# nmoehrle/mvs-texturing

Hardware: AMD Instinct MI355X
Metric: faces/sec through view-selection (data-cost + MRF) (higher is better)
Workload: dtype f32

## Files before the change

### mvs-texturing_amd/csrc/api.hip

```cpp
#include "ctx.h"

#include <atomic>
#include <cmath>
#include <cstdio>
#include <cstdlib>
#include <cstring>
#include <chrono>
#include <mutex>
#include <string>
#include <thread>
#include <vector>

namespace mvs {
void dc_phase1(mvs_ctx* ctx, const mvs_settings* st);
void dc_phase2(mvs_ctx* ctx);
void dc_phase3(mvs_ctx* ctx, mvs_dc_stats* stats);
void undistort_image(mvs_ctx* ctx, const uint8_t* d_src, uint8_t* d_dst, int w, int h, double flen, double d0, double d1);
void dc_prune_labels(mvs_ctx* ctx, uint32_t kmax);
void dc_postprocess(mvs_ctx* ctx, uint32_t nf, uint32_t n_views, const uint32_t* h_ptr, const uint16_t* h_view_rev, const float* h_q_rev, const float* h_col_rev, const mvs_settings* st);
void mrf_setup(mvs_ctx* ctx, const mvs_mrf_params* params);
void mrf_sweep(mvs_ctx* ctx, uint32_t nb0, uint32_t ne0);
void mrf_energy(mvs_ctx* ctx, bool best, uint32_t nb0, uint32_t ne0, bool reduce = true);
void mrf_keep_best(mvs_ctx* ctx);
void mrf_exact_costs(mvs_ctx* ctx, uint32_t nb0, uint32_t ne0);
// ... 311 lines not shown
    if (!ctx) return fail(MVS_ERR_INVALID, "ctx is null");
    MVS_API_BEGIN
    MVS_HIP(hipStreamSynchronize(ctx->stream));
    if (ctx->own_stream && ctx->stream) MVS_HIP(hipStreamDestroy(ctx->stream));
    ctx->stream = (hipStream_t)hip_stream; ctx->own_stream = false;
    MVS_API_END
}

mvs_status mvs_ctx_synchronize(mvs_ctx* ctx) {
    if (!ctx) return fail(MVS_ERR_INVALID, "ctx is null");
    MVS_API_BEGIN
    MVS_HIP(hipStreamSynchronize(ctx->stream));
    MVS_API_END
}

mvs_status mvs_set_option(mvs_ctx* ctx, const char* name, int64_t value) {
    if (!ctx || !name) return fail(MVS_ERR_INVALID, "null argument");
    const std::string n(name);
    if (n == "count_rays") ctx->count_rays = value != 0;
    else if (n == "stats") ctx->stats = value != 0;
    else if (n == "verbose") ctx->verbose = value != 0;
    else if (n == "info_wave_area") ctx->info_wave_area = (int)std::max<int64_t>(0, std::min<int64_t>(value, 1 << 30));
    else if (n == "info_wave_area_words") ctx->info_wave_area_words = (int)std::max<int64_t>(1, std::min<int64_t>(value, 1 << 30));
    else if (n == "info_words") ctx->info_words = value != 0;
    else if (n == "info_cert_shift") ctx->info_cert_shift = (int)std::max<int64_t>(0, std::min<int64_t>(value, 40));
    else if (n == "max_labels") { if (value < 0 || value > 65535) return fail(MVS_ERR_INVALID, "max_labels: 0 (off) .. 65535"); ctx->max_labels = (int)value; }
    else if (n == "profile") ctx->profile = value != 0;
    else if (n == "prep_fused") ctx->prep_fused = value != 0;
    else if (n == "ray_xcd") ctx->ray_xcd = (int)value;
    else if (n == "mrf_xcd") ctx->mrf_xcd = (int)value;
    else if (n == "mrf_lag") ctx->mrf_lag = (int)value;
    else if (n == "shard_peer_push") ctx->shard_peer_push = value != 0;
    else if (n == "mrf_force_generic") ctx->mrf_force_generic = value != 0;
    else if (n == "mrf_wide") ctx->mrf_wide = value != 0;
    else if (n == "mrf_graph") ctx->mrf_graph = value != 0;
    else if (n == "mrf_late_old") ctx->mrf_late_old = (int)value;
    else if (n == "mrf_damp_period") ctx->mrf_damp_period = (int)std::max<int64_t>(0, std::min<int64_t>(value, 64));
    else if (n == "mrf_run_pad") ctx->mrf_run_pad = (value == 16) ? 16 : 4;
    else if (n == "mrf_blocks_per_cu") ctx->mrf_blocks_per_cu = std::max(0, (int)value);
    else if (n == "bvh_caller_order") ctx->bvh_caller_order = value != 0;
    else if (n == "dc_overlap_prep") ctx->dc_overlap_prep = value != 0;
    else if (n == "bvh_upper_min_faces") { ctx->kd_disabled = false; ctx->bvh_upper_min_faces = (uint32_t)std::max<int64_t>(0, std::min<int64_t>(value, 0xFFFFFFFFll)); ctx->order_pinned = false; }
    else if (n == "bvh_window") { ctx->kd_disabled = false; ctx->bvh_window = (uint32_t)std::max<int64_t>(0, std::min<int64_t>(value, 0x40000000)); ctx->order_pinned = false; }
    else if (n == "face_order") { ctx->face_order = value != 0 ? 1 : 0; ctx->order_pinned = false; }
    else return fail(MVS_ERR_INVALID, "unknown option " + n);
    return MVS_OK;
}

mvs_status mvs_ctx_get_profile(mvs_ctx* ctx, char* buf, size_t buf_size) {
    if (!ctx || !buf || buf_size < 3) return fail(MVS_ERR_INVALID, "null argument");
    MVS_API_BEGIN
    MVS_HIP(hipStreamSynchronize(ctx->stream));
    std::vector<std::string> names; std::vector<double> ms; std::vector<int> cnt;
    for (auto& sp : ctx->prof_spans) {
        float t = 0.0f;
        MVS_HIP(hipEventElapsedTime(&t, sp.a, sp.b));
        size_t k = 0;
        for (; k < names.size(); ++k) if (names[k] == sp.name) break;
        if (k == names.size()) { names.push_back(sp.name); ms.push_back(0.0); cnt.push_back(0); }
        ms[k] += t; cnt[k] += 1;
        if (sp.owns_a) ctx->prof_pool.push_back(sp.a);
        ctx->prof_pool.push_back(sp.b);
    }
    ctx->prof_spans.clear();
    std::string out = "{";
    for (size_t k = 0; k < names.size(); ++k) {
// ... 636 lines not shown
```

### mvs-texturing_amd/csrc/ctx.h

```cpp
#pragma once
#include <hip/hip_runtime.h>
#include <stdint.h>
#include <string.h>
#include <algorithm>
#include <stdexcept>
#include <string>
#include <vector>

#include "../../include/mvs_viewsel.h"
#include "dmath.h"

namespace mvs {

struct HipError : std::runtime_error {
    explicit HipError(const std::string& m) : std::runtime_error(m) {}
};
struct StatusError : std::runtime_error {
    mvs_status st;
    StatusError(mvs_status s, const std::string& m) : std::runtime_error(m), st(s) {}
};

#define MVS_HIP(expr)                                                                          \
    do {                                                                                       \
        hipError_t _e = (expr);                                                                \
// ... 157 lines not shown
    const uint32_t* r_ptr = nullptr; const uint16_t* r_view = nullptr; const float* r_cost = nullptr;
    bool csr_q_valid = false;
    bool have_costs = false;
    mvs_settings dc_settings{}; mvs_dc_stats dc_stats{}; int dc_phase = 0;

    mvs::DBuf<unsigned long long> g_keys, g_keys2; mvs::DBuf<uint32_t> g_vals, g_vals2, g_pos, g_cnt, g_adj_ptr, g_adj, g_faces; mvs::DBuf<float> g_normals;
    uint64_t g_adj_entries = 0; bool have_adj = false;

    mvs::DBuf<uint32_t> p_label_ptr, p_comp_ptr, p_comp_faces, p_parent, p_root, p_state, p_flag, p_pos, p_roots, p_roots2, p_rlab, p_rlab2, p_adj_ptr, p_adj, p_labels;

    mvs::DBuf<uint32_t> rg_parent, rg_root, rg_size, rg_bestl, rg_lose, rg_flag, rg_pos, rg_cstart, rg_have, rg_cfirst, rg_name;
    mvs::DBuf<unsigned long long> rg_gain, rg_cur, rg_key, rg_key2, rg_ck, rg_sum; mvs::DBuf<long long> rg_cgain; mvs::DBuf<uint2> rg_cut;

    mvs::DBuf<uint32_t> m_adj_ptr, m_adj, a_stage_ptr, a_stage; const uint32_t* r_adj_ptr = nullptr; const uint32_t* r_adj = nullptr;
    uint32_t r_adj_edges = 0; bool r_adj_edges_known = false;
    mvs::DBuf<mvs::NodeDesc> m_desc; mvs::DBuf<uint8_t> m_ident; mvs::DBuf<uint32_t> m_rec; uint64_t m_rec_words = 0; bool m_fast = false; int mrf_blocks_per_cu = 0 , mrf_xcd = 1, mrf_late_old = 1, mrf_run_pad = 4;
    mvs::DBuf<mvs::MrfEdge> m_edge; mvs::DBuf<uint32_t> m_size, m_rev ; mvs::DBuf<uint16_t> m_map;
    mvs::DBuf<uint8_t> m_msg_a;
    mvs::DBuf<uint32_t> m_sel, m_sel2, m_cand; mvs::DBuf<float> m_gain;
    mvs::DBuf<uint32_t> m_lab; mvs::DBuf<float> m_cost;
    uint32_t m_stride = 0;
    bool exact_valid = false; uint32_t exact_nb = 0, exact_ne = 0;
    uint32_t* b_sel = nullptr; uint32_t* b_lab = nullptr; float* b_cost = nullptr; bool best_resolved = false;
    mvs::DBuf<unsigned long long> m_energy; mvs::DBuf<uint32_t> m_moved; mvs::DBuf<uint32_t> m_alist; bool icm_dirty_valid = false;
    uint32_t m_n_adj = 0;
    uint32_t m_energy_blocks = 0;
    bool m_energy_from_sweep = false;
    uint64_t m_total = 0; uint32_t m_kmax = 0, m_degmax = 0;
    mvs::DBuf<uint32_t> m_colour, m_perm, m_tmp_a, m_tmp_b, m_tmp_c, m_sub; mvs::DBuf<uint8_t> m_cls; uint32_t m_colours = 0, m_n_fast = 0; std::vector<uint32_t> m_sub_begin;
    const uint32_t* m_colour_in = nullptr;
    const uint8_t* m_bnd = nullptr;
    int mrf_damp_period = 4;
    int mrf_force_generic = 0;
    int mrf_wide = 1;
    bool m_wide_layout = false;
    uint32_t m_range_nb = 0, m_range_ne = 0; std::vector<uint32_t> m_range_q;
    uint32_t m_sweep_no = 0;
    mvs_mrf_params m_params{};
    static constexpr uint32_t RING = 16;
    static constexpr uint32_t ICM_RING = 8;
    uint32_t* h_icm = nullptr; uint32_t* d_icm = nullptr; uint32_t icm_seq = 0;
    mvs::DBuf<mvs_mrf_progress> m_state; mvs::DBuf<unsigned long long> m_hist; mvs::DBuf<uint32_t> m_ctl;
    int mrf_graph = 1; hipStream_t cap_stream = nullptr; hipGraphExec_t sweep_exec = nullptr; uint32_t graph_launches = 0, graph_updates = 0, graph_instantiations = 0;
    mvs_mrf_progress* h_ring = nullptr; mvs_mrf_progress* d_ring = nullptr ; uint32_t steps_issued = 0; int mrf_lag = 1;
    int shard_peer_push = 1;
    uint32_t* h_seq = nullptr; uint32_t* d_seq = nullptr; uint32_t seq_base = 0;
};

namespace mvs {
struct Prof {
    mvs_ctx* c; size_t idx; bool on;
    Prof(mvs_ctx* ctx, const char* name) : c(ctx), idx(0), on(ctx->profile) {
        if (!on) return;
        auto get = [&]() { hipEvent_t e; if (!c->prof_pool.empty()) { e = c->prof_pool.back(); c->prof_pool.pop_back(); } else { MVS_HIP(hipEventCreate(&e)); } return e; };
        ProfSpan sp{name, get(), get(), true};
        MVS_HIP(hipEventRecord(sp.a, c->stream));
        idx = c->prof_spans.size(); c->prof_spans.push_back(sp);
    }
    void end() { if (on) { MVS_HIP(hipEventRecord(c->prof_spans[idx].b, c->stream)); on = false; } }
    ~Prof() { if (on) (void)hipEventRecord(c->prof_spans[idx].b, c->stream); }
};
struct ProfChain {
    mvs_ctx* c; hipEvent_t prev; bool on;
    static hipEvent_t get(mvs_ctx* c) { hipEvent_t e; if (!c->prof_pool.empty()) { e = c->prof_pool.back(); c->prof_pool.pop_back(); } else { MVS_HIP(hipEventCreate(&e)); } return e; }
    explicit ProfChain(mvs_ctx* ctx) : c(ctx), prev(nullptr), on(ctx->profile) {}
    void begin() { if (on && !prev) { prev = get(c); MVS_HIP(hipEventRecord(prev, c->stream)); first = true; } }
// ... 22 lines not shown
```

### mvs-texturing_amd/csrc/k_mrf.hip

```cpp
#include "ctx.h"
#include <rocprim/rocprim.hpp>
#include <atomic>

namespace mvs {

namespace {

constexpr uint16_t MAP_NONE = 0xFFFF;
constexpr uint32_t MSG_BASE = MVS_MRF_MSG_BASE;

typedef uint8_t msg_t;
struct MsgQ { float scale, step; };
__device__ __forceinline__ MsgQ msg_q(float lam) { return MsgQ{255.0f / lam, lam / 255.0f}; }
template <class T> __device__ __forceinline__ T ld_off(const void* base, uint32_t byte_off) { return *reinterpret_cast<const T*>(reinterpret_cast<const char*>(base) + byte_off); }
template <class T> __device__ __forceinline__ void st_off(void* base, uint32_t byte_off, T v) { *reinterpret_cast<T*>(reinterpret_cast<char*>(base) + byte_off) = v; }
__device__ __forceinline__ float min_raw(float a, float b) { float r; asm("v_min_f32 %0, %1, %2" : "=v"(r) : "v"(a), "v"(b)); return r; }
template <bool DAMP>
__device__ __forceinline__ uint32_t msg_pack_s(float raw_s, float alpha, float old_code, uint32_t byte, uint32_t word) {
    return __builtin_amdgcn_cvt_pk_u8_f32(DAMP ? __builtin_fmaf(old_code, alpha, raw_s) : raw_s, byte, word);
}
template <bool DAMP>
__device__ __forceinline__ uint32_t msg_pack(float raw, float oms, float alpha, float old_code, uint32_t byte, uint32_t word) {
    const float v = DAMP ? __builtin_fmaf(old_code, alpha, raw * oms) : raw * oms;
    return __builtin_amdgcn_cvt_pk_u8_f32(v, byte, word);
// ... 318 lines not shown
}

__global__ void __launch_bounds__(256) mrf_ident_kernel(const uint32_t* __restrict__ col_ptr, const uint16_t* __restrict__ view_id, const uint32_t* __restrict__ adj_ptr,
                                                        const uint32_t* __restrict__ adj, uint32_t F, const MrfEdge* __restrict__ edge, const uint8_t* __restrict__ cls,
                                                        uint8_t* __restrict__ ident) {
    const uint32_t i = (blockIdx.x * blockDim.x + threadIdx.x) >> 4;
    const uint32_t gl = threadIdx.x & 15;
    if (i >= F || cls[i] == CLS_GENERIC) return;
    const uint32_t p0 = col_ptr[i], K = col_ptr[i + 1] - p0;
    const uint32_t e0 = adj_ptr[i], e1 = adj_ptr[i + 1];
    for (uint32_t e = e0; e < e1; e += 3) {
        uint32_t kj[3], q0[3];
#pragma unroll
        for (int k = 0; k < 3; ++k) {
            const bool on = e + k < e1;
            kj[k] = on ? edge[e + k].kj : 0u;
            q0[k] = col_ptr[on ? adj[e + k] : i];
        }
        uint32_t same = 0;
#pragma unroll
        for (int k = 0; k < 3; ++k) same |= (kj[k] != 0u && kj[k] == K) ? (1u << k) : 0u;
        if (same) {
            for (uint32_t t = gl; t < K; t += 16) {
                const uint32_t v = view_id[p0 + t];
#pragma unroll
                for (int k = 0; k < 3; ++k)
                    if ((same >> k) & 1u) { if (view_id[q0[k] + t] != v) same &= ~(1u << k); }
            }
            for (int o = 8; o > 0; o >>= 1) same &= __shfl_xor(same, o, 16);
        }
        if (gl < 3 && e + gl < e1 && kj[gl] != 0u) ident[e + gl] = (uint8_t)((same >> gl) & 1u);
    }
}
__global__ void mrf_recsize_kernel(const uint32_t* __restrict__ col_ptr, const uint32_t* __restrict__ adj_ptr, const MrfEdge* __restrict__ edge,
                                   const uint8_t* __restrict__ ident, const uint8_t* __restrict__ cls, const uint32_t* __restrict__ perm, uint32_t F, uint32_t wide,
                                   uint32_t* __restrict__ rsz, uint32_t* __restrict__ qpos) {
    const uint32_t q = blockIdx.x * blockDim.x + threadIdx.x;
    if (q > F) return;
    uint32_t w = 0;
    if (q < F) {
        const uint32_t i = perm[q], K = col_ptr[i + 1] - col_ptr[i];
        qpos[i] = q;
        if (K && cls[i] != CLS_GENERIC) {
            w = (K + 3u) & ~3u;
            const bool w8 = wide != 0u && cls[i] == 1u;
            const uint32_t e0 = adj_ptr[i], e1 = adj_ptr[i + 1];
            for (uint32_t eb = e0; eb < e1; eb += 4) {
                uint32_t kj[4], id[4];
#pragma unroll
                for (int t = 0; t < 4; ++t) { const bool on = eb + t < e1; kj[t] = on ? edge[eb + t].kj : 0u; id[t] = on ? ident[eb + t] : 1u; }
#pragma unroll
                for (int t = 0; t < 4; ++t) if (kj[t] && !id[t]) w += w8 ? 2u * ((kj[t] + 7u) >> 3) : (kj[t] + 3u) >> 2;
            }
            w = (w + 3u) & ~3u;
        }
    }
    rsz[q] = w;
}
__global__ void __launch_bounds__(256) mrf_record_kernel(const uint32_t* __restrict__ col_ptr, const uint16_t* __restrict__ view_id, const float* __restrict__ cost,
                                                         const uint32_t* __restrict__ adj_ptr, const uint32_t* __restrict__ adj, const MrfEdge* __restrict__ edge,
                                                         const uint8_t* __restrict__ ident, const uint8_t* __restrict__ cls, const uint32_t* __restrict__ qpos, const uint32_t* __restrict__ roff,
                                                         uint32_t F, uint32_t wide, uint32_t* __restrict__ rec) {
    __shared__ uint16_t s_l[16][256];
    const uint32_t i = (blockIdx.x * blockDim.x + threadIdx.x) >> 4;
    const uint32_t gl = threadIdx.x & 15;
    if (i >= F) return;
    const uint32_t p0 = col_ptr[i], K = col_ptr[i + 1] - p0;
    const uint32_t ci = cls[i];
    if (K == 0 || ci == CLS_GENERIC) return;
    const bool w8 = wide != 0u && ci == 1u;
    const uint32_t rs = w8 ? 8u : 8u << ci, none_byte = w8 ? 64u : (ci < 3u ? 4u * rs : 0xFFu);
    const uint32_t lmask = w8 ? 7u : 3u, lshift = w8 ? 3u : 2u;
    const uint32_t q = qpos[i];
    uint16_t* tile = s_l[threadIdx.x >> 4];
    uint32_t* out = rec + REC_BASE + roff[q];
    const uint32_t K4 = (K + 3u) & ~3u;
    const uint32_t e0 = adj_ptr[i], deg = adj_ptr[i + 1] - e0;
    uint32_t kj3[3], q03[3];
    {
        uint32_t kj[3], idn[3], nb[3];
#pragma unroll
        for (uint32_t d = 0; d < 3; ++d) { const bool on = d < deg; kj[d] = on ? edge[e0 + d].kj : 0u; idn[d] = on ? (uint32_t)ident[e0 + d] : 1u; nb[d] = on ? adj[e0 + d] : i; }
#pragma unroll
// ... 595 lines not shown
        bool stop = false;
        if ((int)sw >= min_sweeps && (int)sw > window) {
            const unsigned long long prev = hist[sw - (uint32_t)window];
            stop = (double)(prev - p.best) < (double)min_improvement * (double)prev;
        }
        if ((int)sw >= max_sweeps) stop = true;
        if (stop) { p.stopped = 1u; p.stop_sweep = sw; }
    }
    *st = p;
    const uint32_t n = ctl[0] + 1u; ctl[0] = n;
    if (ring) {
        const uint32_t slot = n % ring_slots;
        ring[slot] = p;
        __threadfence_system();
        __hip_atomic_store(ring_seq + slot, ctl[1] + n, __ATOMIC_RELEASE, __HIP_MEMORY_SCOPE_SYSTEM);
    }
}
__global__ void report_u32_kernel(const uint32_t* __restrict__ src, uint32_t* __restrict__ dst, uint32_t* __restrict__ dst_seq, uint32_t seq) {
    *dst = *src;
    __threadfence_system();
    __hip_atomic_store(dst_seq, seq, __ATOMIC_RELEASE, __HIP_MEMORY_SCOPE_SYSTEM);
}
__global__ void report_words_kernel(const uint32_t* __restrict__ src, uint32_t n, uint32_t* __restrict__ dst, uint32_t* __restrict__ dst_seq, uint32_t seq) {
    if (threadIdx.x < n) dst[threadIdx.x] = src[threadIdx.x];
    __threadfence_system();
    __syncthreads();
    if (threadIdx.x == 0) __hip_atomic_store(dst_seq, seq, __ATOMIC_RELEASE, __HIP_MEMORY_SCOPE_SYSTEM);
}
__global__ void mrf_flip_kernel(mvs_mrf_progress* __restrict__ st) { st->best_w = st->w; st->w ^= 1u; }

}

constexpr uint32_t EPART_BLOCKS = 2048;

void mrf_setup(mvs_ctx* ctx, const mvs_mrf_params* params) {
    hipStream_t s = ctx->stream;
    const uint32_t F = ctx->csr_faces;
    ctx->m_params = *params;
    if (!(params->rho > 0.0f && params->rho <= 1.0f) || !(params->damping >= 0.0f && params->damping < 1.0f))
        throw StatusError(MVS_ERR_INVALID, "mrf params: need 0 < rho <= 1, 0 <= damping < 1");
    if (params->window < 1 || params->min_sweeps < 0 || !(params->min_improvement >= 0.0f) || params->icm_iters < 0)
        throw StatusError(MVS_ERR_INVALID, "mrf params: need window >= 1, min_sweeps >= 0, min_improvement >= 0, icm_iters >= 0");
    uint32_t E = ctx->r_adj_edges;
    if (!ctx->r_adj_edges_known) {
        MVS_HIP(hipMemcpyAsync(&E, ctx->r_adj_ptr + F, sizeof(uint32_t), hipMemcpyDeviceToHost, s));
        MVS_HIP(hipStreamSynchronize(s));
    }
    ctx->m_size.ensure((size_t)E + 2); ctx->m_edge.ensure((size_t)E + 1); ctx->m_moved.ensure(8 + 2 * 64);
    ctx->m_n_adj = E;
    uint32_t* maxes = ctx->m_moved.p + 4;
    MVS_HIP(hipMemsetAsync(ctx->m_moved.p, 0, 8 * sizeof(uint32_t), s));
    MVS_HIP(hipMemsetAsync(ctx->m_size.p, 0, ((size_t)E + 2) * sizeof(uint32_t), s));
    const unsigned nb = (F + 255) / 256;
    const uint32_t force_generic = (ctx->csr_nnz < 4 || E == 0 || ctx->mrf_force_generic) ? 1u : 0u;
    ctx->m_cls.ensure((size_t)F + 4);
    ctx->m_rev.ensure((size_t)E + 2);
    if (F) { hipLaunchKernelGGL(mrf_size_kernel, dim3(nb), dim3(256), 0, s, ctx->r_ptr, ctx->r_adj_ptr, ctx->r_adj, F, (uint32_t)(ctx->mrf_run_pad == 16 ? 15 : (ctx->mrf_wide ? 7 : 3)), force_generic, ctx->m_size.p, ctx->m_cls.p, maxes, ctx->m_rev.p); MVS_LAUNCH_CHECK(); }
    ctx->m_colour.ensure((size_t)F + 2); ctx->m_perm.ensure((size_t)F + 2); ctx->m_tmp_a.ensure((size_t)MAX_LAYOUT_COLOURS * ((size_t)F + 1) + 72); ctx->m_tmp_b.ensure((size_t)MAX_LAYOUT_COLOURS * ((size_t)F + 1) + 2); ctx->m_tmp_c.ensure((size_t)F + 2);
    ctx->m_colours = 0; ctx->m_sub_begin.assign(N_KEY + 1, 0); ctx->m_n_fast = 0; ctx->m_range_q.clear(); ctx->m_range_nb = ctx->m_range_ne = 0;
    ctx->m_sweep_no = 0;
    if (F) {
        uint32_t* pending = ctx->m_moved.p + 1;
        hipLaunchKernelGGL(mrf_colour_init_kernel, dim3(nb), dim3(256), 0, s, ctx->m_colour.p, ctx->m_tmp_a.p , F); MVS_LAUNCH_CHECK();
        if (ctx->m_colour_in) MVS_HIP(hipMemcpyAsync(ctx->m_colour.p, ctx->m_colour_in, (size_t)F * sizeof(uint32_t), hipMemcpyDeviceToDevice, s));
        for (int round = 0; !ctx->m_colour_in; ++round) {
            if (round >= 4096) throw StatusError(MVS_ERR_HIP, "graph colouring did not terminate");
            MVS_HIP(hipMemsetAsync(pending, 0, sizeof(uint32_t), s));
            for (int k = 0; k < (round == 0 ? 16 : 4); ++k) { hipLaunchKernelGGL(mrf_colour_round_kernel, dim3(nb), dim3(256), 0, s, ctx->r_adj_ptr, ctx->r_adj, ctx->t_perm, F, ctx->m_colour.p, pending); MVS_LAUNCH_CHECK(); }
            uint32_t hp[2] = {0, 0};
            read_words(ctx, pending, hp, 2);
            if (hp[1]) throw StatusError(MVS_ERR_UNSUPPORTED, "adjacency graph needs more than 64 colours (a node with >= 64 mutually constrained neighbours)");
            if (!hp[0]) break;
        }
        MVS_HIP(hipMemsetAsync(ctx->m_moved.p, 0, 4 * sizeof(uint32_t), s));
        hipLaunchKernelGGL(mrf_sortkey_kernel, dim3(nb), dim3(256), 0, s, ctx->m_colour.p, ctx->m_cls.p, ctx->m_bnd, F, ctx->m_tmp_c.p); MVS_LAUNCH_CHECK();
        size_t tmp_bytes = 0;
        MVS_HIP(rocprim::radix_sort_pairs(nullptr, tmp_bytes, ctx->m_tmp_c.p, ctx->m_tmp_b.p, ctx->m_tmp_a.p, ctx->m_perm.p, F, 0, 10, s));
        ctx->sort_tmp.ensure(tmp_bytes + 16);
        MVS_HIP(rocprim::radix_sort_pairs(ctx->sort_tmp.p, tmp_bytes, ctx->m_tmp_c.p, ctx->m_tmp_b.p, ctx->m_tmp_a.p, ctx->m_perm.p, F, 0, 10, s));
        ctx->m_sub.ensure(3 * (size_t)N_KEY + 8);
        hipLaunchKernelGGL(mrf_sub_begin_kernel, dim3((N_KEY + 256) / 256), dim3(256), 0, s, ctx->m_tmp_b.p, F, ctx->m_sub.p); MVS_LAUNCH_CHECK();
        read_block(ctx, ctx->m_sub.p, ctx->m_sub_begin.data(), (N_KEY + 1) * sizeof(uint32_t));
        const std::vector<uint32_t>& sb = ctx->m_sub_begin;
        uint32_t C = 0;
        for (uint32_t c = 0; c < 64; ++c) if (sb[2 * (4 * c + 4)] > sb[2 * (4 * c)] || sb[2 * (SUB_GENERIC + c + 1)] > sb[2 * (SUB_GENERIC + c)]) C = c + 1;
        ctx->m_colours = C;
        ctx->m_n_fast = sb[2 * SUB_GENERIC];
    }
    DBuf<uint32_t>& in_off = ctx->m_sel2;
    in_off.ensure(std::max<size_t>((size_t)E + 2, (size_t)F + 2));
    MVS_HIP(hipMemsetAsync(in_off.p, 0, ((size_t)E + 2) * sizeof(uint32_t), s));
    uint32_t h[3] = {0, 0, 0};
    if (F) {
        if ((uint64_t)E * 4ull + 4ull * (uint64_t)ctx->csr_nnz >= 0xFFFFFFF0ull) {
            const uint64_t total = sum_u32(ctx, ctx->m_size.p, (size_t)E + 1);
            if ((uint64_t)MSG_BASE + total >= 0xFFFFFFF0ull) throw StatusError(MVS_ERR_UNSUPPORTED, "message array exceeds 2^32 elements (shard the graph: DESIGN.md multi-GPU)");
        }
        const uint32_t n_col = (ctx->m_colours >= 2 && ctx->m_colours <= (uint32_t)MAX_LAYOUT_COLOURS) ? ctx->m_colours : 1u;
        const size_t n_ent = (size_t)n_col * ((size_t)F + 1);
        ctx->m_tmp_a.ensure(n_ent + 72); ctx->m_tmp_b.ensure(n_ent + 2);
        hipLaunchKernelGGL(mrf_nodesize_kernel, dim3((F + 256) / 256), dim3(256), 0, s, ctx->m_perm.p, ctx->m_colour.p, ctx->r_adj_ptr, ctx->r_adj, ctx->m_size.p, ctx->m_rev.p, F, n_col, ctx->m_tmp_a.p); MVS_LAUNCH_CHECK();
        exclusive_scan_u32(ctx, ctx->m_tmp_a.p, ctx->m_tmp_b.p, n_ent, nullptr);
        hipLaunchKernelGGL(mrf_inoff_kernel, dim3(nb), dim3(256), 0, s, ctx->m_perm.p, ctx->m_colour.p, ctx->r_adj_ptr, ctx->r_adj, ctx->m_size.p, ctx->m_rev.p, ctx->m_tmp_b.p, F, n_col, in_off.p); MVS_LAUNCH_CHECK();
        MVS_HIP(hipMemcpyAsync(maxes + 2, ctx->m_tmp_b.p + (n_ent - 1), sizeof(uint32_t), hipMemcpyDeviceToDevice, s));
    } else MVS_HIP(hipMemsetAsync(maxes + 2, 0, sizeof(uint32_t), s));
    { uint32_t hm[3]; read_words(ctx, maxes, hm, 3); h[1] = hm[0]; h[2] = hm[1]; h[0] = hm[2]; }
    ctx->m_total = (uint64_t)MSG_BASE + h[0]; ctx->m_kmax = h[1]; ctx->m_degmax = h[2];
    if (ctx->m_total >= 0xFFFFFFF0ull) throw StatusError(MVS_ERR_UNSUPPORTED, "message array exceeds 2^32 elements");
    if (F) { hipLaunchKernelGGL(mrf_edge_kernel, dim3(nb), dim3(256), 0, s, ctx->r_ptr, ctx->r_adj_ptr, ctx->r_adj, F, in_off.p, ctx->m_size.p, ctx->m_rev.p, ctx->m_edge.p); MVS_LAUNCH_CHECK(); }
    ctx->m_ident.ensure((size_t)E + 1);
    MVS_HIP(hipMemsetAsync(ctx->m_ident.p, 0, (size_t)E + 1, s));
    ctx->m_fast = true;
    ctx->m_wide_layout = ctx->mrf_wide != 0;
    const uint32_t n_fast = ctx->m_n_fast, n_generic = F - n_fast;
    if (n_fast) {
        const size_t rec_cap = (size_t)REC_BASE + ctx->csr_nnz + 8 * (size_t)F + ctx->m_total / 4 + (ctx->mrf_wide ? (size_t)ctx->m_n_adj : 0) + 1024;
        ctx->m_rec.ensure(rec_cap);
        MVS_HIP(hipMemsetAsync(ctx->m_rec.p, 0, REC_BASE * sizeof(uint32_t), s));
        hipLaunchKernelGGL(mrf_ident_kernel, dim3((unsigned)(((size_t)F * 16 + 255) / 256)), dim3(256), 0, s, ctx->r_ptr, ctx->r_view, ctx->r_adj_ptr, ctx->r_adj, F, ctx->m_edge.p, ctx->m_cls.p, ctx->m_ident.p); MVS_LAUNCH_CHECK();
        uint32_t* rsz = ctx->m_tmp_a.p; uint32_t* roff = ctx->m_tmp_b.p;
        hipLaunchKernelGGL(mrf_recsize_kernel, dim3((F + 256) / 256), dim3(256), 0, s, ctx->r_ptr, ctx->r_adj_ptr, ctx->m_edge.p, ctx->m_ident.p, ctx->m_cls.p, ctx->m_perm.p, F, (uint32_t)(ctx->mrf_wide ? 1 : 0), rsz, ctx->m_tmp_c.p); MVS_LAUNCH_CHECK();
        exclusive_scan_u32(ctx, rsz, roff, (size_t)F + 1, nullptr);
        hipLaunchKernelGGL(mrf_record_kernel, dim3((unsigned)(((size_t)F * 16 + 255) / 256)), dim3(256), 0, s, ctx->r_ptr, ctx->r_view, ctx->r_cost, ctx->r_adj_ptr, ctx->r_adj,
                           ctx->m_edge.p, ctx->m_ident.p, ctx->m_cls.p, ctx->m_tmp_c.p , roff, F, (uint32_t)(ctx->mrf_wide ? 1 : 0), ctx->m_rec.p); MVS_LAUNCH_CHECK();
        ctx->m_desc.ensure((size_t)F + 1);
        hipLaunchKernelGGL(mrf_desc_kernel, dim3((n_fast + 255) / 256), dim3(256), 0, s, ctx->r_ptr, ctx->r_adj_ptr, ctx->r_adj, ctx->m_edge.p, ctx->m_ident.p, ctx->m_perm.p, ctx->m_colour.p, roff, n_fast, ctx->m_desc.p); MVS_LAUNCH_CHECK();
    }
    if (n_generic) {
        ctx->m_map.ensure(ctx->m_total + 8);
        hipLaunchKernelGGL(mrf_map_kernel, dim3((unsigned)(((size_t)F * 16 + 255) / 256)), dim3(256), 0, s, ctx->r_ptr, ctx->r_view, ctx->r_adj_ptr, ctx->r_adj, F, ctx->m_edge.p, ctx->m_cls.p, ctx->m_map.p); MVS_LAUNCH_CHECK();
        ctx->pq.ensure(ctx->csr_nnz + 1);
    }
    ctx->m_msg_a.ensure(ctx->m_total + 1024);
    MVS_HIP(hipMemsetAsync(ctx->m_msg_a.p, 0, (ctx->m_total + 1024) * sizeof(msg_t), s));
    const size_t F1 = (size_t)F + 1;
    ctx->m_stride = (uint32_t)F1;
    ctx->m_sel.ensure(2 * F1); ctx->m_lab.ensure(2 * F1); ctx->m_cost.ensure(2 * F1);
    ctx->m_sel2.ensure(F1); ctx->m_cand.ensure(F1); ctx->m_gain.ensure(F1);
    MVS_HIP(hipMemsetAsync(ctx->m_sel.p, 0, 2 * F1 * sizeof(uint32_t), s));
    MVS_HIP(hipMemsetAsync(ctx->m_lab.p, 0, 2 * F1 * sizeof(uint32_t), s));
    MVS_HIP(hipMemsetAsync(ctx->m_cost.p, 0, 2 * F1 * sizeof(float), s));
    mvs_mrf_progress init; memset(&init, 0, sizeof(init)); init.best = ~0ull; init.energy = ~0ull; init.w = 0u; init.best_w = 1u;
    if (F && params->max_sweeps <= 0) {
        hipLaunchKernelGGL(mrf_argmin_unary_kernel, dim3(nb), dim3(256), 0, s, ctx->r_ptr, ctx->r_view, ctx->r_cost, F, ctx->m_sel.p, ctx->m_lab.p, ctx->m_cost.p);
        MVS_LAUNCH_CHECK();
        init.w = 1u; init.best_w = 0u;
    }
    ctx->b_sel = ctx->m_sel.p + init.best_w * F1; ctx->b_lab = ctx->m_lab.p + init.best_w * F1; ctx->b_cost = ctx->m_cost.p + init.best_w * F1;
    ctx->best_resolved = true;
    MVS_HIP(hipMemsetAsync(ctx->m_gain.p, 0, F1 * sizeof(float), s));
    const size_t epart = 4 + 2 * (size_t)EPART_BLOCKS * std::max<size_t>(ctx->m_colours, 1);
    ctx->m_energy.ensure(epart);
    MVS_HIP(hipMemsetAsync(ctx->m_energy.p, 0, epart * sizeof(unsigned long long), s));
    ctx->m_state.ensure(1); ctx->m_hist.ensure((size_t)std::max(params->max_sweeps, 0) + 2);
// ... 209 lines not shown
    for (int k = 0; k < n; ++k) {
        const unsigned cap = slot_end - slot - (unsigned)(n - 1 - k);
        const uint32_t qb = L[k].qb, qe = L[k].qe;
        switch (L[k].g) {
            case 0: slot += launch_sweep4_g<8>(ctx, phase, qb, qe, slot, cap); break;
            case 1: slot += ctx->m_wide_layout ? launch_sweep8(ctx, phase, qb, qe, slot, cap) : launch_sweep4_g<16>(ctx, phase, qb, qe, slot, cap); break;
            case 2: slot += launch_sweep4_g<32>(ctx, phase, qb, qe, slot, cap); break;
            case 3: slot += launch_sweep4_g<64>(ctx, phase, qb, qe, slot, cap); break;
            default: slot += launch_sweep_generic(ctx, phase, qb, qe, slot, cap);
        }
    }
}
void mrf_sweep(mvs_ctx* ctx, uint32_t nb0, uint32_t ne0) {
    for (uint32_t ph = 0; ph < ctx->m_colours; ++ph) mrf_sweep_phase(ctx, ph, nb0, ne0, MRF_PART_ALL);
    ctx->m_energy_from_sweep = nb0 == 0 && ne0 >= ctx->csr_faces && ctx->m_colours > 0;
}

__global__ void mrf_exact_cost_kernel(const uint32_t* __restrict__ col_ptr, const uint16_t* __restrict__ view_id, const float* __restrict__ cost,
                                      const uint32_t* __restrict__ lab, uint32_t node_begin, uint32_t node_end, uint32_t* __restrict__ sel, float* __restrict__ selcost,
                                      uint32_t* __restrict__ foreign ) {
    const uint32_t i = node_begin + blockIdx.x * blockDim.x + threadIdx.x;
    if (i >= node_end) return;
    const uint32_t p0 = col_ptr[i], K = col_ptr[i + 1] - p0, l = lab[i];
    const uint32_t t = (K && l) ? label_position(view_id, p0, K, l) : 0u;
    if ((K != 0u) != (l != 0u) || (K && l && (uint32_t)view_id[p0 + t] + 1u != l)) atomicAdd(foreign, 1u);
    sel[i] = t;
    selcost[i] = K ? cost[p0 + t] : 1.0f;
}
void mrf_exact_costs(mvs_ctx* ctx, uint32_t nb0, uint32_t ne0) {
    resolve_best(ctx);
    if (ne0 <= nb0) return;
    if (ctx->exact_valid && ctx->exact_nb == nb0 && ctx->exact_ne == ne0) return;
    ctx->exact_valid = true; ctx->exact_nb = nb0; ctx->exact_ne = ne0;
    MVS_HIP(hipMemsetAsync(ctx->m_moved.p + 6, 0, sizeof(uint32_t), ctx->stream));
    hipLaunchKernelGGL(mrf_exact_cost_kernel, dim3((ne0 - nb0 + 255) / 256), dim3(256), 0, ctx->stream, ctx->r_ptr, ctx->r_view, ctx->r_cost, (const uint32_t*)ctx->b_lab, nb0, ne0, ctx->b_sel, ctx->b_cost, ctx->m_moved.p + 6);
    MVS_LAUNCH_CHECK();
}

void mrf_energy(mvs_ctx* ctx, bool best, uint32_t nb0, uint32_t ne0, bool reduce) {
    const unsigned blocks = ne0 > nb0 ? std::min<unsigned>((ne0 - nb0 + 255) / 256, 2048u) : 0u;
    ctx->m_energy_blocks = blocks; ctx->m_energy_from_sweep = false;
    unsigned long long* partial = ctx->m_energy.p + 4;
    if (best) mrf_exact_costs(ctx, nb0, ne0);
    if (blocks) {
        if (best) hipLaunchKernelGGL(mrf_energy_kernel, dim3(blocks), dim3(256), 0, ctx->stream, ctx->r_ptr, ctx->r_view, ctx->r_cost, ctx->r_adj_ptr, ctx->r_adj, ctx->b_lab, ctx->b_cost, (const mvs_mrf_progress*)nullptr, 0u, nb0, ne0, partial);
        else hipLaunchKernelGGL(mrf_energy_kernel, dim3(blocks), dim3(256), 0, ctx->stream, ctx->r_ptr, ctx->r_view, ctx->r_cost, ctx->r_adj_ptr, ctx->r_adj, ctx->m_lab.p, ctx->m_cost.p, ctx->m_state.p, ctx->m_stride, nb0, ne0, partial);
        MVS_LAUNCH_CHECK();
    }
    if (!reduce) return;
    hipLaunchKernelGGL(mrf_energy_reduce_kernel, dim3(1), dim3(1024), 0, ctx->stream, partial, blocks, ctx->m_energy.p, (unsigned long long*)nullptr);
    MVS_LAUNCH_CHECK();
}
void mrf_sweep_energy_reduce(mvs_ctx* ctx, unsigned long long* out2) {
    const uint32_t n = EPART_BLOCKS * std::max<uint32_t>(ctx->m_colours, 1u);
    hipLaunchKernelGGL(mrf_energy_reduce_kernel, dim3(1), dim3(1024), 0, ctx->stream, ctx->m_energy.p + 4, n, ctx->m_energy.p, out2);
    MVS_LAUNCH_CHECK();
}

void mrf_keep_best(mvs_ctx* ctx) {
    ctx->icm_dirty_valid = false; ctx->best_resolved = false; ctx->exact_valid = false;
    if (!ctx->m_state.p) throw StatusError(MVS_ERR_STATE, "mrf setup first");
    hipLaunchKernelGGL(mrf_flip_kernel, dim3(1), dim3(1), 0, ctx->stream, ctx->m_state.p);
    MVS_LAUNCH_CHECK();
}

void mrf_icm_gain(mvs_ctx* ctx, uint32_t nb0, uint32_t ne0) {
    if (ne0 <= nb0) return;
    resolve_best(ctx);
// ... 18 lines not shown
            if (K <= 8) ICM_D(8); else if (K <= 64) ICM_D(16); else ICM_D(32);
#undef ICM_D
            MVS_LAUNCH_CHECK();
        }
        if (nf < n) ICM_G(64, nf, n, (const uint32_t*)ctx->m_perm.p);
    } else {
        const uint32_t* none = nullptr;
        if (K <= 8) ICM_G(8, nb0, ne0, none); else if (K <= 64) ICM_G(16, nb0, ne0, none); else if (K <= 128) ICM_G(32, nb0, ne0, none); else ICM_G(64, nb0, ne0, none);
    }
#undef ICM_G
    MVS_LAUNCH_CHECK();
    ctx->icm_dirty_valid = whole;
}
void mrf_icm_apply(mvs_ctx* ctx, uint32_t nb0, uint32_t ne0) {
    MVS_HIP(hipMemsetAsync(ctx->m_moved.p, 0, 2 * sizeof(uint32_t), ctx->stream));
    if (ne0 <= nb0) return;
    resolve_best(ctx);
    const bool whole = nb0 == 0 && ne0 == ctx->csr_faces;
    if (!whole) ctx->icm_dirty_valid = false;
    uint32_t* alist = nullptr;
    if (ctx->icm_dirty_valid) {
        ctx->m_alist.ensure((size_t)ctx->csr_faces + (size_t)ctx->m_n_adj + 16);
        alist = ctx->m_alist.p;
    }
    hipLaunchKernelGGL(mrf_icm_apply_kernel, dim3((ne0 - nb0 + 255) / 256), dim3(256), 0, ctx->stream, ctx->r_ptr, ctx->r_view, ctx->r_cost, ctx->r_adj_ptr, ctx->r_adj,
                       ctx->m_gain.p, ctx->m_cand.p, ctx->b_sel, ctx->b_lab, ctx->b_cost, nb0, ne0, ctx->m_moved.p, alist, ctx->t_perm);
    MVS_LAUNCH_CHECK();
}
void mrf_labels(mvs_ctx* ctx, uint32_t nb0, uint32_t ne0, uint32_t* d_labels, uint32_t out[2], bool caller_order) {
    uint32_t* bu = ctx->m_moved.p + 2;
    resolve_best(ctx);
    MVS_HIP(hipMemsetAsync(bu, 0, 2 * sizeof(uint32_t), ctx->stream));
    if (ne0 > nb0) {
        const uint32_t* foreign = (ctx->exact_valid && ctx->exact_nb == nb0 && ctx->exact_ne == ne0) ? ctx->m_moved.p + 6 : (const uint32_t*)nullptr;
        hipLaunchKernelGGL(mrf_labels_kernel, dim3((ne0 - nb0 + 255) / 256), dim3(256), 0, ctx->stream, ctx->b_lab, nb0, ne0, ctx->csr_views, d_labels, bu, caller_order ? ctx->t_perm : (const uint32_t*)nullptr, foreign);
        MVS_LAUNCH_CHECK();
    }
    read_words(ctx, bu, out, 2);
}

}
```

Measured before the change: 75.42 million.

## Replace per-edge label-set comparison with per-face view bitmaps in MRF setup

Adds a kernel that builds a per-face bitmap of candidate views (when there are at most 256 views and each face's views are strictly sorted), then computes edge identity in the record-size kernel by comparing neighbour bitmaps instead of running the gather-based ident kernel. This drops the memset of the ident array and, when the bitmap is valid, the ident kernel itself. The goal is to cut setup cost from comparing sorted view lists element by element on every edge. In exchange it adds a bitmap pass and an extra host readback word, keeps a fallback to the old ident kernel when the ordering check fails, and moves the foreign-label counter slot from index 6 to index 8.

```diff
diff --git a/mvs-texturing_amd/csrc/api.hip b/mvs-texturing_amd/csrc/api.hip
--- a/mvs-texturing_amd/csrc/api.hip
+++ b/mvs-texturing_amd/csrc/api.hip
@@ -367,6 +367,7 @@
     else if (n == "mrf_lag") ctx->mrf_lag = (int)value;
     else if (n == "shard_peer_push") ctx->shard_peer_push = value != 0;
     else if (n == "mrf_force_generic") ctx->mrf_force_generic = value != 0;
+    else if (n == "mrf_ident_gather") ctx->mrf_ident_gather = value != 0;
     else if (n == "mrf_wide") ctx->mrf_wide = value != 0;
     else if (n == "mrf_graph") ctx->mrf_graph = value != 0;
     else if (n == "mrf_late_old") ctx->mrf_late_old = (int)value;
diff --git a/mvs-texturing_amd/csrc/ctx.h b/mvs-texturing_amd/csrc/ctx.h
--- a/mvs-texturing_amd/csrc/ctx.h
+++ b/mvs-texturing_amd/csrc/ctx.h
@@ -213,6 +213,8 @@
     const uint8_t* m_bnd = nullptr;
     int mrf_damp_period = 4;
     int mrf_force_generic = 0;
+    mvs::DBuf<uint32_t> m_bits;
+    int mrf_ident_gather = 0;
     int mrf_wide = 1;
     bool m_wide_layout = false;
     uint32_t m_range_nb = 0, m_range_ne = 0; std::vector<uint32_t> m_range_q;
diff --git a/mvs-texturing_amd/csrc/k_mrf.hip b/mvs-texturing_amd/csrc/k_mrf.hip
--- a/mvs-texturing_amd/csrc/k_mrf.hip
+++ b/mvs-texturing_amd/csrc/k_mrf.hip
@@ -374,8 +374,56 @@
         if (gl < 3 && e + gl < e1 && kj[gl] != 0u) ident[e + gl] = (uint8_t)((same >> gl) & 1u);
     }
 }
-__global__ void mrf_recsize_kernel(const uint32_t* __restrict__ col_ptr, const uint32_t* __restrict__ adj_ptr, const MrfEdge* __restrict__ edge,
-                                   const uint8_t* __restrict__ ident, const uint8_t* __restrict__ cls, const uint32_t* __restrict__ perm, uint32_t F, uint32_t wide,
+template <int WS>
+__global__ void __launch_bounds__(256) mrf_bitmap_kernel(const uint32_t* __restrict__ col_ptr, const uint16_t* __restrict__ view_id, uint32_t F,
+                                                         uint32_t* __restrict__ bits, uint32_t* __restrict__ bad) {
+    const uint32_t i = (blockIdx.x * blockDim.x + threadIdx.x) >> 3;
+    const uint32_t gl = threadIdx.x & 7;
+    if (i >= F) return;
+    const uint32_t p0 = col_ptr[i], K = col_ptr[i + 1] - p0;
+    uint32_t acc[WS];
+#pragma unroll
+    for (int w = 0; w < WS; ++w) acc[w] = 0u;
+    bool ok = true;
+    for (uint32_t t0 = 0; t0 < K; t0 += 64) {
+        uint32_t v[8], nx[8];
+#pragma unroll
+        for (int u = 0; u < 8; ++u) {
+            const uint32_t t = t0 + 8u * u + gl;
+            v[u] = (t < K) ? (uint32_t)view_id[p0 + t] : 0u;
+            nx[u] = (t + 1u < K) ? (uint32_t)view_id[p0 + t + 1u] : 0x10000u;
+        }
+#pragma unroll
+        for (int u = 0; u < 8; ++u) {
+            if (t0 + 8u * u + gl >= K) continue;
+            if (nx[u] <= v[u] || v[u] >= 32u * WS) ok = false;
+#pragma unroll
+            for (int w = 0; w < WS; ++w) acc[w] |= ((v[u] >> 5) == (uint32_t)w) ? (1u << (v[u] & 31u)) : 0u;
+        }
+    }
+    uint32_t mine = 0u;
+#pragma unroll
+    for (int w = 0; w < WS; ++w) {
+        uint32_t a = acc[w];
+        a |= dpp_u<0xB1>(a); a |= dpp_u<0x4E>(a); a |= dpp_u<0x141>(a);
+        mine = (gl == (uint32_t)w) ? a : mine;
+    }
+    if (gl < (uint32_t)WS) bits[(size_t)i * WS + gl] = mine;
+    if (!ok) *bad = 1u;
+}
+template <int WS>
+__device__ __forceinline__ void load_bits(const uint32_t* __restrict__ p, uint32_t (&b)[WS]) {
+    if constexpr (WS == 1) b[0] = p[0];
+    else if constexpr (WS == 2) { const uint2 v = *reinterpret_cast<const uint2*>(p); b[0] = v.x; b[1] = v.y; }
+    else {
+#pragma unroll
+        for (int h = 0; h < WS / 4; ++h) { const uint4 v = reinterpret_cast<const uint4*>(p)[h]; b[4 * h] = v.x; b[4 * h + 1] = v.y; b[4 * h + 2] = v.z; b[4 * h + 3] = v.w; }
+    }
+}
+
+template <int WS>
+__global__ void mrf_recsize_kernel(const uint32_t* __restrict__ col_ptr, const uint32_t* __restrict__ adj_ptr, const uint32_t* __restrict__ adj, const MrfEdge* __restrict__ edge,
+                                   uint8_t* __restrict__ ident, const uint32_t* __restrict__ bits, const uint8_t* __restrict__ cls, const uint32_t* __restrict__ perm, uint32_t F, uint32_t wide,
                                    uint32_t* __restrict__ rsz, uint32_t* __restrict__ qpos) {
     const uint32_t q = blockIdx.x * blockDim.x + threadIdx.x;
     if (q > F) return;
@@ -387,10 +435,30 @@
             w = (K + 3u) & ~3u;
             const bool w8 = wide != 0u && cls[i] == 1u;
             const uint32_t e0 = adj_ptr[i], e1 = adj_ptr[i + 1];
+            constexpr int WB = WS > 0 ? WS : 1;
+            uint32_t bi[WB];
+            if constexpr (WS > 0) load_bits<WS>(bits + (size_t)i * WS, bi);
             for (uint32_t eb = e0; eb < e1; eb += 4) {
                 uint32_t kj[4], id[4];
-#pragma unroll
-                for (int t = 0; t < 4; ++t) { const bool on = eb + t < e1; kj[t] = on ? edge[eb + t].kj : 0u; id[t] = on ? ident[eb + t] : 1u; }
+                if constexpr (WS > 0) {
+                    uint32_t j[4];
+#pragma unroll
+                    for (int t = 0; t < 4; ++t) { const bool on = eb + t < e1; kj[t] = on ? edge[eb + t].kj : 0u; j[t] = on ? adj[eb + t] : i; }
+                    uint32_t bj[4][WB];
+#pragma unroll
+                    for (int t = 0; t < 4; ++t) load_bits<WS>(bits + (size_t)j[t] * WS, bj[t]);
+#pragma unroll
+                    for (int t = 0; t < 4; ++t) {
+                        bool same = kj[t] == K;
+#pragma unroll
+                        for (int x = 0; x < WS; ++x) same = same && bj[t][x] == bi[x];
+                        id[t] = same ? 1u : 0u;
+                        if (kj[t]) ident[eb + t] = (uint8_t)id[t];
+                    }
+                } else {
+#pragma unroll
+                    for (int t = 0; t < 4; ++t) { const bool on = eb + t < e1; kj[t] = on ? edge[eb + t].kj : 0u; id[t] = on ? ident[eb + t] : 1u; }
+                }
 #pragma unroll
                 for (int t = 0; t < 4; ++t) if (kj[t] && !id[t]) w += w8 ? 2u * ((kj[t] + 7u) >> 3) : (kj[t] + 3u) >> 2;
             }
@@ -1052,6 +1120,7 @@
 }
 
 constexpr uint32_t EPART_BLOCKS = 2048;
+constexpr uint32_t W_FOREIGN = 8;
 
 void mrf_setup(mvs_ctx* ctx, const mvs_mrf_params* params) {
     hipStream_t s = ctx->stream;
@@ -1076,6 +1145,16 @@
     ctx->m_cls.ensure((size_t)F + 4);
     ctx->m_rev.ensure((size_t)E + 2);
     if (F) { hipLaunchKernelGGL(mrf_size_kernel, dim3(nb), dim3(256), 0, s, ctx->r_ptr, ctx->r_adj_ptr, ctx->r_adj, F, (uint32_t)(ctx->mrf_run_pad == 16 ? 15 : (ctx->mrf_wide ? 7 : 3)), force_generic, ctx->m_size.p, ctx->m_cls.p, maxes, ctx->m_rev.p); MVS_LAUNCH_CHECK(); }
+    const uint32_t V = ctx->csr_views;
+    const uint32_t ws = (F && ctx->csr_nnz && !force_generic && !ctx->mrf_ident_gather && V <= 256u) ? (V <= 32u ? 1u : V <= 64u ? 2u : V <= 128u ? 4u : 8u) : 0u;
+    if (ws) {
+        ctx->m_bits.ensure((size_t)F * ws + 8);
+        const dim3 g((unsigned)(((size_t)F * 8 + 255) / 256));
+#define MRF_BITMAP(W) hipLaunchKernelGGL(mrf_bitmap_kernel<W>, g, dim3(256), 0, s, ctx->r_ptr, ctx->r_view, F, ctx->m_bits.p, maxes + 3)
+        if (ws == 1) MRF_BITMAP(1); else if (ws == 2) MRF_BITMAP(2); else if (ws == 4) MRF_BITMAP(4); else MRF_BITMAP(8);
+#undef MRF_BITMAP
+        MVS_LAUNCH_CHECK();
+    }
     ctx->m_colour.ensure((size_t)F + 2); ctx->m_perm.ensure((size_t)F + 2); ctx->m_tmp_a.ensure((size_t)MAX_LAYOUT_COLOURS * ((size_t)F + 1) + 72); ctx->m_tmp_b.ensure((size_t)MAX_LAYOUT_COLOURS * ((size_t)F + 1) + 2); ctx->m_tmp_c.ensure((size_t)F + 2);
     ctx->m_colours = 0; ctx->m_sub_begin.assign(N_KEY + 1, 0); ctx->m_n_fast = 0; ctx->m_range_q.clear(); ctx->m_range_nb = ctx->m_range_ne = 0;
     ctx->m_sweep_no = 0;
@@ -1124,12 +1203,12 @@
         hipLaunchKernelGGL(mrf_inoff_kernel, dim3(nb), dim3(256), 0, s, ctx->m_perm.p, ctx->m_colour.p, ctx->r_adj_ptr, ctx->r_adj, ctx->m_size.p, ctx->m_rev.p, ctx->m_tmp_b.p, F, n_col, in_off.p); MVS_LAUNCH_CHECK();
         MVS_HIP(hipMemcpyAsync(maxes + 2, ctx->m_tmp_b.p + (n_ent - 1), sizeof(uint32_t), hipMemcpyDeviceToDevice, s));
     } else MVS_HIP(hipMemsetAsync(maxes + 2, 0, sizeof(uint32_t), s));
-    { uint32_t hm[3]; read_words(ctx, maxes, hm, 3); h[1] = hm[0]; h[2] = hm[1]; h[0] = hm[2]; }
+    bool bits_ok = false;
+    { uint32_t hm[4]; read_words(ctx, maxes, hm, 4); h[1] = hm[0]; h[2] = hm[1]; h[0] = hm[2]; bits_ok = ws != 0u && hm[3] == 0u; }
     ctx->m_total = (uint64_t)MSG_BASE + h[0]; ctx->m_kmax = h[1]; ctx->m_degmax = h[2];
     if (ctx->m_total >= 0xFFFFFFF0ull) throw StatusError(MVS_ERR_UNSUPPORTED, "message array exceeds 2^32 elements");
     if (F) { hipLaunchKernelGGL(mrf_edge_kernel, dim3(nb), dim3(256), 0, s, ctx->r_ptr, ctx->r_adj_ptr, ctx->r_adj, F, in_off.p, ctx->m_size.p, ctx->m_rev.p, ctx->m_edge.p); MVS_LAUNCH_CHECK(); }
     ctx->m_ident.ensure((size_t)E + 1);
-    MVS_HIP(hipMemsetAsync(ctx->m_ident.p, 0, (size_t)E + 1, s));
     ctx->m_fast = true;
     ctx->m_wide_layout = ctx->mrf_wide != 0;
     const uint32_t n_fast = ctx->m_n_fast, n_generic = F - n_fast;
@@ -1137,9 +1216,14 @@
         const size_t rec_cap = (size_t)REC_BASE + ctx->csr_nnz + 8 * (size_t)F + ctx->m_total / 4 + (ctx->mrf_wide ? (size_t)ctx->m_n_adj : 0) + 1024;
         ctx->m_rec.ensure(rec_cap);
         MVS_HIP(hipMemsetAsync(ctx->m_rec.p, 0, REC_BASE * sizeof(uint32_t), s));
-        hipLaunchKernelGGL(mrf_ident_kernel, dim3((unsigned)(((size_t)F * 16 + 255) / 256)), dim3(256), 0, s, ctx->r_ptr, ctx->r_view, ctx->r_adj_ptr, ctx->r_adj, F, ctx->m_edge.p, ctx->m_cls.p, ctx->m_ident.p); MVS_LAUNCH_CHECK();
+        if (!bits_ok) { hipLaunchKernelGGL(mrf_ident_kernel, dim3((unsigned)(((size_t)F * 16 + 255) / 256)), dim3(256), 0, s, ctx->r_ptr, ctx->r_view, ctx->r_adj_ptr, ctx->r_adj, F, ctx->m_edge.p, ctx->m_cls.p, ctx->m_ident.p); MVS_LAUNCH_CHECK(); }
         uint32_t* rsz = ctx->m_tmp_a.p; uint32_t* roff = ctx->m_tmp_b.p;
-        hipLaunchKernelGGL(mrf_recsize_kernel, dim3((F + 256) / 256), dim3(256), 0, s, ctx->r_ptr, ctx->r_adj_ptr, ctx->m_edge.p, ctx->m_ident.p, ctx->m_cls.p, ctx->m_perm.p, F, (uint32_t)(ctx->mrf_wide ? 1 : 0), rsz, ctx->m_tmp_c.p); MVS_LAUNCH_CHECK();
+        const uint32_t rws = bits_ok ? ws : 0u;
+#define MRF_RECSIZE(W) hipLaunchKernelGGL(mrf_recsize_kernel<W>, dim3((F + 256) / 256), dim3(256), 0, s, ctx->r_ptr, ctx->r_adj_ptr, ctx->r_adj, ctx->m_edge.p, ctx->m_ident.p, \
+                                          (const uint32_t*)ctx->m_bits.p, ctx->m_cls.p, ctx->m_perm.p, F, (uint32_t)(ctx->mrf_wide ? 1 : 0), rsz, ctx->m_tmp_c.p)
+        if (rws == 0) MRF_RECSIZE(0); else if (rws == 1) MRF_RECSIZE(1); else if (rws == 2) MRF_RECSIZE(2); else if (rws == 4) MRF_RECSIZE(4); else MRF_RECSIZE(8);
+#undef MRF_RECSIZE
+        MVS_LAUNCH_CHECK();
         exclusive_scan_u32(ctx, rsz, roff, (size_t)F + 1, nullptr);
         hipLaunchKernelGGL(mrf_record_kernel, dim3((unsigned)(((size_t)F * 16 + 255) / 256)), dim3(256), 0, s, ctx->r_ptr, ctx->r_view, ctx->r_cost, ctx->r_adj_ptr, ctx->r_adj,
                            ctx->m_edge.p, ctx->m_ident.p, ctx->m_cls.p, ctx->m_tmp_c.p , roff, F, (uint32_t)(ctx->mrf_wide ? 1 : 0), ctx->m_rec.p); MVS_LAUNCH_CHECK();
@@ -1415,8 +1499,8 @@
     if (ne0 <= nb0) return;
     if (ctx->exact_valid && ctx->exact_nb == nb0 && ctx->exact_ne == ne0) return;
     ctx->exact_valid = true; ctx->exact_nb = nb0; ctx->exact_ne = ne0;
-    MVS_HIP(hipMemsetAsync(ctx->m_moved.p + 6, 0, sizeof(uint32_t), ctx->stream));
-    hipLaunchKernelGGL(mrf_exact_cost_kernel, dim3((ne0 - nb0 + 255) / 256), dim3(256), 0, ctx->stream, ctx->r_ptr, ctx->r_view, ctx->r_cost, (const uint32_t*)ctx->b_lab, nb0, ne0, ctx->b_sel, ctx->b_cost, ctx->m_moved.p + 6);
+    MVS_HIP(hipMemsetAsync(ctx->m_moved.p + W_FOREIGN, 0, sizeof(uint32_t), ctx->stream));
+    hipLaunchKernelGGL(mrf_exact_cost_kernel, dim3((ne0 - nb0 + 255) / 256), dim3(256), 0, ctx->stream, ctx->r_ptr, ctx->r_view, ctx->r_cost, (const uint32_t*)ctx->b_lab, nb0, ne0, ctx->b_sel, ctx->b_cost, ctx->m_moved.p + W_FOREIGN);
     MVS_LAUNCH_CHECK();
 }
 
@@ -1501,7 +1585,7 @@
     resolve_best(ctx);
     MVS_HIP(hipMemsetAsync(bu, 0, 2 * sizeof(uint32_t), ctx->stream));
     if (ne0 > nb0) {
-        const uint32_t* foreign = (ctx->exact_valid && ctx->exact_nb == nb0 && ctx->exact_ne == ne0) ? ctx->m_moved.p + 6 : (const uint32_t*)nullptr;
+        const uint32_t* foreign = (ctx->exact_valid && ctx->exact_nb == nb0 && ctx->exact_ne == ne0) ? ctx->m_moved.p + W_FOREIGN : (const uint32_t*)nullptr;
         hipLaunchKernelGGL(mrf_labels_kernel, dim3((ne0 - nb0 + 255) / 256), dim3(256), 0, ctx->stream, ctx->b_lab, nb0, ne0, ctx->csr_views, d_labels, bu, caller_order ? ctx->t_perm : (const uint32_t*)nullptr, foreign);
         MVS_LAUNCH_CHECK();
     }
```

After: 75.99 million, median of 6. Within noise of the previous version (+0.8%).
